# mathwrx/Decouple-and-Couple_Learning_in_Multi-Modal_Brain_Tumor_Segmentation

Measured on AMD Instinct MI355X. Metric: training volumes/sec (4x128^3), higher is better.
Workload: dtype bf16x3 forward (split-bf16 MFMA operands hi.hi+hi.lo+lo.hi: logits within 1e-3 of the fp32 reference) / bf16 data-gradient / bf16 weight-gradient MFMA operands; f32 accumulate, f32 storage, f32 master weights; 1 GPU; configs[1]: 1xMI355X, batch 2 per GPU, 4-modality 128^3 synthetic BraTS patches; fwd + softmax_dice + 4 sub-region/edge losses + bwd + Adam(amsgrad); random-init weights, dropout on; global_batch=2, parallelism=dp1, precision=bf16x3, dgrad_precision=bf16, wgrad_precision=bf16, mode=plan

## Files before the change

decouple-and-couple_learning_in_multi-modal_brain_tumor_segmentation_amd/csrc/gemm.hip:

```cpp
#include "common.h"
#include <cstdlib>

typedef struct cwf_gemm_args GemmArgs;


template <int TM, int TN, int GK>
__global__ __launch_bounds__(256) void gemm_mfma_kernel(const GemmArgs a) {
  constexpr int LDA_S = GK + 1, LDB_S = TN + 16;
  constexpr int IM = TM / 32, JN = TN / 32;
  constexpr int SA = TM * GK / 256, SB = TN * GK / 256;
  __shared__ float As[TM * LDA_S];
  __shared__ float Bs[GK * LDB_S];
  const int tid = threadIdx.x, lane = tid & 63, wave = tid >> 6;
  const int wr = wave >> 1, wc = wave & 1;
  const int r = lane & 15, kq = lane >> 4;
  const int zb = blockIdx.z / a.ZH, zh = blockIdx.z % a.ZH;
  const int m0 = blockIdx.y * TM, n0 = blockIdx.x * TN;
  const int64_t a_zoff = zb * a.sa_zb + zh * a.sa_zh;
  const float* A = ((a.A2 && n0 >= a.split_n) ? a.A2 : a.A) + a_zoff;
  const bool tabB = a.B_tab[0] != nullptr;
  const float* B = tabB ? a.B_tab[blockIdx.z] : a.B + zb * a.sb_zb + zh * a.sb_zh;
  if (a.B2 && m0 >= a.split_m) B = a.B2 + zb * a.sb_zb + zh * a.sb_zh;
  const bool a_drop = a.a_drop_p > 0.f;
  float* rowsum = a.rowsum_tab[0] ? a.rowsum_tab[blockIdx.z] : a.rowsum;
  const bool do_rs = rowsum != nullptr && blockIdx.x == 0 && wc == 0;

  f32x4 acc[IM][JN], accr[IM];
#pragma unroll
  for (int i = 0; i < IM; ++i) {
    accr[i] = (f32x4){0.f, 0.f, 0.f, 0.f};
#pragma unroll
    for (int j = 0; j < JN; ++j) acc[i][j] = (f32x4){0.f, 0.f, 0.f, 0.f};
  }

  const bool a_kfast = (a.sa_k == 1);
  const bool b_nfast = (a.sb_n == 1);
  int am[SA], ak[SA], bk[SB], bn[SB];
#pragma unroll
  for (int i = 0; i < SA; ++i) {
    if (a_kfast) { ak[i] = tid % GK; am[i] = tid / GK + (256 / GK) * i; } else { am[i] = tid % TM; ak[i] = tid / TM + (256 / TM) * i; }
  }
#pragma unroll
  for (int i = 0; i < SB; ++i) {
    if (b_nfast) { bn[i] = tid % TN; bk[i] = tid / TN + (256 / TN) * i; } else { bk[i] = tid % GK; bn[i] = tid / GK + (256 / GK) * i; }
  }
  float ra[SA], rb[SB];
  auto fetch = [&](int k0) {
#pragma unroll
    for (int i = 0; i < SA; ++i) {
      const int gm = m0 + am[i], gk = k0 + ak[i];
      float v = 0.f;
      if (gm < a.M && gk < a.K) {
        const int64_t off = gm * a.sa_m + gk * a.sa_k;
        v = A[off];
        if (a_drop) v *= cwf_keep(a.rng, a.a_drop_off, (uint64_t)(a_zoff + off), a.a_drop_n, a.a_drop_p, a.a_drop_p2);
      }
      ra[i] = v;
    }
#pragma unroll
    for (int i = 0; i < SB; ++i) {
      const int gn = n0 + bn[i], gkb = k0 + bk[i];
      rb[i] = (gn < a.N && gkb < a.K) ? B[gkb * a.sb_k + gn * a.sb_n] : 0.f;
    }
  };
  fetch(0);
  for (int k0 = 0; k0 < a.K; k0 += GK) {
    if (k0) __syncthreads();
#pragma unroll
    for (int i = 0; i < SA; ++i) As[am[i] * LDA_S + ak[i]] = ra[i];
#pragma unroll
    for (int i = 0; i < SB; ++i) Bs[bk[i] * LDB_S + bn[i]] = rb[i];
    __syncthreads();
    if (k0 + GK < a.K) fetch(k0 + GK);
#pragma unroll
    for (int kk = 0; kk < GK / 4; ++kk) {
      float av[IM], bv[JN];
#pragma unroll
      for (int i = 0; i < IM; ++i) av[i] = As[(wr * (TM / 2) + i * 16 + r) * LDA_S + kk * 4 + kq];
#pragma unroll
      for (int j = 0; j < JN; ++j) bv[j] = Bs[(kk * 4 + kq) * LDB_S + wc * (TN / 2) + j * 16 + r];
#pragma unroll
      for (int i = 0; i < IM; ++i)
#pragma unroll
        for (int j = 0; j < JN; ++j) acc[i][j] = __builtin_amdgcn_mfma_f32_16x16x4f32(av[i], bv[j], acc[i][j], 0, 0, 0);
      if (do_rs) {
#pragma unroll
        for (int i = 0; i < IM; ++i) accr[i] = __builtin_amdgcn_mfma_f32_16x16x4f32(av[i], 1.0f, accr[i], 0, 0, 0);
      }
    }
  }
  const int64_t c_zoff = zb * a.sc_zb + zh * a.sc_zh;
  float* C = a.C_tab[0] ? a.C_tab[blockIdx.z] : a.C + c_zoff;
  float* C2 = a.C2 ? a.C2 + c_zoff : nullptr;
  const float* bias = a.bias_tab[0] ? a.bias_tab[blockIdx.z] : a.bias;
  const float* R = a.residual ? a.residual + zb * a.sr_zb + zh * a.sr_zh : nullptr;
  const bool c_drop = a.c_drop_p > 0.f;
#pragma unroll
  for (int i = 0; i < IM; ++i)
#pragma unroll
    for (int j = 0; j < JN; ++j) {
      const int gn = n0 + wc * (TN / 2) + j * 16 + r;
      if (gn >= a.N) continue;
      const float bv = bias ? bias[gn] : 0.f;
#pragma unroll
      for (int e = 0; e < 4; ++e) {
        const int gm = m0 + wr * (TM / 2) + i * 16 + kq * 4 + e;
        if (gm >= a.M) continue;
        const int64_t off = gm * a.sc_m + gn;
        float v = acc[i][j][e] * a.alpha + bv;
        if (C2) C2[off] = v;
        if (a.act == 1) v = 0.5f * v * (1.f + erff(v * 0.70710678118654752440f));
        if (c_drop) v *= cwf_keep(a.rng, a.c_drop_off, (uint64_t)(c_zoff + off), a.c_drop_n, a.c_drop_p, a.c_drop_p2);
        if (R) v += R[gm * a.sr_m + gn];
        float* p = C + off;
        if (a.accumulate) v += *p;
        *p = v;
      }
    }
  if (do_rs && r == 0) {
#pragma unroll
    for (int i = 0; i < IM; ++i)
#pragma unroll
      for (int e = 0; e < 4; ++e) {
        const int gm = m0 + wr * (TM / 2) + i * 16 + kq * 4 + e;
        if (gm < a.M) rowsum[gm] = (a.rowsum_acc ? rowsum[gm] : 0.f) + accr[i][e];
      }
  }
}

template <int TM, int TN, int GK, bool AK, bool BN>
__global__ __launch_bounds__(256) void gemm_mfma_v_kernel(const GemmArgs a) {
  constexpr int LDA_S = GK + 1, LDB_S = TN + 16;
  constexpr int IM = TM / 32, JN = TN / 32;
  constexpr int SA = TM * GK / 1024, SB = TN * GK / 1024;
  __shared__ float As[TM * LDA_S];
  __shared__ __attribute__((aligned(16))) float Bs[GK * LDB_S];
  const int tid = threadIdx.x, lane = tid & 63, wave = tid >> 6;
  const int wr = wave >> 1, wc = wave & 1;
  const int r = lane & 15, kq = lane >> 4;
  const int zb = blockIdx.z / a.ZH, zh = blockIdx.z % a.ZH;
  const int m0 = blockIdx.y * TM, n0 = blockIdx.x * TN;
  const int64_t a_zoff = zb * a.sa_zb + zh * a.sa_zh;
  const float* A = ((a.A2 && n0 >= a.split_n) ? a.A2 : a.A) + a_zoff;
  const bool tabB = a.B_tab[0] != nullptr;
  const float* B = tabB ? a.B_tab[blockIdx.z] : a.B + zb * a.sb_zb + zh * a.sb_zh;
  if (a.B2 && m0 >= a.split_m) B = a.B2 + zb * a.sb_zb + zh * a.sb_zh;
  const bool a_drop = a.a_drop_p > 0.f;
  float* rowsum = a.rowsum_tab[0] ? a.rowsum_tab[blockIdx.z] : a.rowsum;
  const bool do_rs = rowsum != nullptr && blockIdx.x == 0 && wc == 0;

  f32x4 acc[IM][JN], accr[IM];
#pragma unroll
  for (int i = 0; i < IM; ++i) {
    accr[i] = (f32x4){0.f, 0.f, 0.f, 0.f};
#pragma unroll
    for (int j = 0; j < JN; ++j) acc[i][j] = (f32x4){0.f, 0.f, 0.f, 0.f};
  }
  int am[SA], ak[SA], bk[SB], bn[SB];
#pragma unroll
  for (int i = 0; i < SA; ++i) {
    if (AK) { ak[i] = (tid % (GK / 4)) * 4; am[i] = tid / (GK / 4) + (1024 / GK) * i; }
    else { am[i] = (tid % (TM / 4)) * 4; ak[i] = tid / (TM / 4) + (1024 / TM) * i; }
  }
#pragma unroll
  for (int i = 0; i < SB; ++i) {
    if (BN) { bn[i] = (tid % (TN / 4)) * 4; bk[i] = tid / (TN / 4) + (1024 / TN) * i; }
    else { bk[i] = (tid % (GK / 4)) * 4; bn[i] = tid / (GK / 4) + (1024 / GK) * i; }
  }
  f32x4 ra[SA], rb[SB];
  auto fetch = [&](int k0) {
#pragma unroll
    for (int i = 0; i < SA; ++i) {
      const int gm = m0 + am[i], gk = k0 + ak[i];
      f32x4 v = {0.f, 0.f, 0.f, 0.f};
      if (gm < a.M && gk < a.K) {
        const int64_t off = gm * a.sa_m + gk * a.sa_k;
        v = *reinterpret_cast<const f32x4*>(A + off);
        if (a_drop) {
          const int64_t st = AK ? 1 : a.sa_m;
#pragma unroll
          for (int c = 0; c < 4; ++c) v[c] *= cwf_keep(a.rng, a.a_drop_off, (uint64_t)(a_zoff + off + c * st), a.a_drop_n, a.a_drop_p, a.a_drop_p2);
        }
      }
      ra[i] = v;
    }
#pragma unroll
    for (int i = 0; i < SB; ++i) {
      const int gn = n0 + bn[i], gkb = k0 + bk[i];
      rb[i] = (gn < a.N && gkb < a.K) ? *reinterpret_cast<const f32x4*>(B + gkb * a.sb_k + gn * a.sb_n) : (f32x4){0.f, 0.f, 0.f, 0.f};
    }
  };
  fetch(0);
  for (int k0 = 0; k0 < a.K; k0 += GK) {
    if (k0) __syncthreads();
#pragma unroll
    for (int i = 0; i < SA; ++i)
#pragma unroll
      for (int c = 0; c < 4; ++c) {
        if (AK) As[am[i] * LDA_S + ak[i] + c] = ra[i][c];
        else As[(am[i] + c) * LDA_S + ak[i]] = ra[i][c];
      }
#pragma unroll
    for (int i = 0; i < SB; ++i) {
      if (BN) *reinterpret_cast<f32x4*>(&Bs[bk[i] * LDB_S + bn[i]]) = rb[i];
      else {
#pragma unroll
        for (int c = 0; c < 4; ++c) Bs[(bk[i] + c) * LDB_S + bn[i]] = rb[i][c];
      }
    }
    __syncthreads();
    if (k0 + GK < a.K) fetch(k0 + GK);
#pragma unroll
    for (int kk = 0; kk < GK / 4; ++kk) {
      float av[IM], bv[JN];
#pragma unroll
      for (int i = 0; i < IM; ++i) av[i] = As[(wr * (TM / 2) + i * 16 + r) * LDA_S + kk * 4 + kq];
#pragma unroll
      for (int j = 0; j < JN; ++j) bv[j] = Bs[(kk * 4 + kq) * LDB_S + wc * (TN / 2) + j * 16 + r];
#pragma unroll
      for (int i = 0; i < IM; ++i)
#pragma unroll
        for (int j = 0; j < JN; ++j) acc[i][j] = __builtin_amdgcn_mfma_f32_16x16x4f32(av[i], bv[j], acc[i][j], 0, 0, 0);
      if (do_rs) {
#pragma unroll
        for (int i = 0; i < IM; ++i) accr[i] = __builtin_amdgcn_mfma_f32_16x16x4f32(av[i], 1.0f, accr[i], 0, 0, 0);
      }
    }
  }
  const int64_t c_zoff = zb * a.sc_zb + zh * a.sc_zh;
  float* C = a.C_tab[0] ? a.C_tab[blockIdx.z] : a.C + c_zoff;
  float* C2 = a.C2 ? a.C2 + c_zoff : nullptr;
  const float* bias = a.bias_tab[0] ? a.bias_tab[blockIdx.z] : a.bias;
  const float* R = a.residual ? a.residual + zb * a.sr_zb + zh * a.sr_zh : nullptr;
  const bool c_drop = a.c_drop_p > 0.f;
#pragma unroll
  for (int i = 0; i < IM; ++i)
#pragma unroll
    for (int j = 0; j < JN; ++j) {
      const int gn = n0 + wc * (TN / 2) + j * 16 + r;
      if (gn >= a.N) continue;
      const float bv = bias ? bias[gn] : 0.f;
#pragma unroll
      for (int e = 0; e < 4; ++e) {
        const int gm = m0 + wr * (TM / 2) + i * 16 + kq * 4 + e;
        if (gm >= a.M) continue;
        const int64_t off = gm * a.sc_m + gn;
        float v = acc[i][j][e] * a.alpha + bv;
        if (C2) C2[off] = v;
        if (a.act == 1) v = 0.5f * v * (1.f + erff(v * 0.70710678118654752440f));
        if (c_drop) v *= cwf_keep(a.rng, a.c_drop_off, (uint64_t)(c_zoff + off), a.c_drop_n, a.c_drop_p, a.c_drop_p2);
        if (R) v += R[gm * a.sr_m + gn];
        float* p = C + off;
        if (a.accumulate) v += *p;
        *p = v;
      }
    }
  if (do_rs && r == 0) {
#pragma unroll
    for (int i = 0; i < IM; ++i)
#pragma unroll
      for (int e = 0; e < 4; ++e) {
        const int gm = m0 + wr * (TM / 2) + i * 16 + kq * 4 + e;
        if (gm < a.M) rowsum[gm] = (a.rowsum_acc ? rowsum[gm] : 0.f) + accr[i][e];
      }
  }
}

static bool gemm_vec_ok(const GemmArgs& a, bool* ak, bool* bn) {
  auto al = [](const void* p) { return (reinterpret_cast<uintptr_t>(p) & 15) == 0; };
  auto m4 = [](int64_t v) { return (v & 3) == 0; };
  if (!m4(a.sa_zb) || !m4(a.sa_zh) || !m4(a.sb_zb) || !m4(a.sb_zh)) return false;
  if (!al(a.A) || (a.A2 && !al(a.A2)) || (a.B && !al(a.B)) || (a.B2 && !al(a.B2))) return false;
  for (int z = 0; z < 4; ++z)
    if (a.B_tab[z] && !al(a.B_tab[z])) return false;
  if (a.sa_k == 1 && m4(a.K) && m4(a.sa_m)) *ak = true;
  else if (a.sa_m == 1 && m4(a.M) && m4(a.sa_k)) *ak = false;
  else return false;
  if (a.sb_n == 1 && m4(a.N) && m4(a.sb_k)) *bn = true;
  else if (a.sb_k == 1 && m4(a.K) && m4(a.sb_n)) *bn = false;
  else return false;
  if (a.B2 && (a.split_m & 3)) return false;
  return true;
}

struct GemmVariant { bool vec; int tm; bool ak, bn; };
static GemmVariant gemm_variant(const GemmArgs& a) {
  const int64_t wg64 = (int64_t)cdiv(a.N, 64) * cdiv(a.M, 64) * a.ZB * a.ZH;
  GemmVariant v = {false, wg64 >= 256 ? 64 : 32, false, false};
  if (a.K >= 64 && gemm_vec_ok(a, &v.ak, &v.bn)) v.vec = true;
  else v.ak = v.bn = false;
  return v;
}

static int gemm_check(const GemmArgs& a) {
  if (!a.A || (!a.B && !a.B_tab[0]) || (!a.C && !a.C_tab[0]) || a.M <= 0 || a.N <= 0 || a.K <= 0 || a.ZB <= 0 || a.ZH <= 0) return CWF_E_BADARG;
  if ((a.B_tab[0] || a.bias_tab[0] || a.C_tab[0] || a.rowsum_tab[0]) && (a.ZH != 1 || a.ZB > 4)) return CWF_E_BADARG;
  if ((int64_t)a.ZB * a.ZH > 65535) return CWF_E_TOOLARGE;
  if ((a.A2 && (a.split_n & 63)) || (a.B2 && (a.split_m & 63))) return CWF_E_BADARG;
  if ((a.a_drop_p > 0.f || a.c_drop_p > 0.f) && !a.rng) return CWF_E_BADARG;
  if (a.rowsum && (int64_t)a.ZB * a.ZH != 1) return CWF_E_BADARG;
  for (int z = 0; z < a.ZB && z < 4; ++z)
    if ((a.B_tab[0] && !a.B_tab[z]) || (a.bias_tab[0] && !a.bias_tab[z]) || (a.C_tab[0] && !a.C_tab[z]) || (a.rowsum_tab[0] && !a.rowsum_tab[z])) return CWF_E_BADARG;
  return 0;
}

extern "C" int cwf_gemm_ex(const struct cwf_gemm_args* args, void* stream) {
  if (!args) return CWF_E_BADARG;
  const GemmArgs& a = *args;
  const int rc = gemm_check(a);
  if (rc) return rc;
  const GemmVariant v = gemm_variant(a);
  const bool big = v.tm == 64;
  if (v.vec) {
    dim3 grid(cdiv(a.N, big ? 64 : 32), cdiv(a.M, big ? 64 : 32), a.ZB * a.ZH);
#define CWF_GV(AKv, BNv) do { if (big) hipLaunchKernelGGL((gemm_mfma_v_kernel<64, 64, 32, AKv, BNv>), grid, dim3(256), 0, cwf_stream(stream), a); \
                              else hipLaunchKernelGGL((gemm_mfma_v_kernel<32, 32, 64, AKv, BNv>), grid, dim3(256), 0, cwf_stream(stream), a); } while (0)
    if (v.ak && v.bn) CWF_GV(true, true); else if (v.ak) CWF_GV(true, false); else if (v.bn) CWF_GV(false, true); else CWF_GV(false, false);
#undef CWF_GV
    CWF_LAUNCH_CHECK();
    return 0;
  }
  if (big) {
    dim3 grid(cdiv(a.N, 64), cdiv(a.M, 64), a.ZB * a.ZH);
    hipLaunchKernelGGL((gemm_mfma_kernel<64, 64, 32>), grid, dim3(256), 0, cwf_stream(stream), a);
  } else {
    dim3 grid(cdiv(a.N, 32), cdiv(a.M, 32), a.ZB * a.ZH);
    hipLaunchKernelGGL((gemm_mfma_kernel<32, 32, 32>), grid, dim3(256), 0, cwf_stream(stream), a);
  }
  CWF_LAUNCH_CHECK();
  return 0;
}

extern "C" int cwf_debug_gemm_variant(const struct cwf_gemm_args* args, int* out) {
  if (!args || !out) return CWF_E_BADARG;
  const int rc = gemm_check(*args);
  if (rc) return rc;
  const GemmVariant v = gemm_variant(*args);
  out[0] = v.vec; out[1] = v.tm; out[2] = v.ak; out[3] = v.bn;
  return 0;
}

extern "C" int cwf_gemm(const float* A, int64_t sa_m, int64_t sa_k, int64_t sa_zb, int64_t sa_zh,
                        const float* B, int64_t sb_k, int64_t sb_n, int64_t sb_zb, int64_t sb_zh,
                        float* C, int64_t sc_m, int64_t sc_zb, int64_t sc_zh,
                        const float* bias, const float* residual, int64_t sr_m, int64_t sr_zb, int64_t sr_zh,
                        int M, int Nn, int K, int ZB, int ZH, float alpha, int act, int accumulate, void* stream) {
  GemmArgs a = {};
  a.A = A; a.sa_m = sa_m; a.sa_k = sa_k; a.sa_zb = sa_zb; a.sa_zh = sa_zh;
  a.B = B; a.sb_k = sb_k; a.sb_n = sb_n; a.sb_zb = sb_zb; a.sb_zh = sb_zh;
  a.C = C; a.sc_m = sc_m; a.sc_zb = sc_zb; a.sc_zh = sc_zh;
  a.bias = bias; a.residual = residual; a.sr_m = sr_m; a.sr_zb = sr_zb; a.sr_zh = sr_zh;
  a.M = M; a.N = Nn; a.K = K; a.ZB = ZB; a.ZH = ZH; a.alpha = alpha; a.act = act; a.accumulate = accumulate;
  return cwf_gemm_ex(&a, stream);
}

template <int PER>
__global__ __launch_bounds__(256) void layernorm_fwd_kernel(const float* __restrict__ x, const float* __restrict__ gamma, const float* __restrict__ beta,
                                                           float* __restrict__ y, float* __restrict__ mean, float* __restrict__ rstd, int rows, int E, float eps) {
  const int row = blockIdx.x * 4 + (threadIdx.x >> 6), lane = threadIdx.x & 63;
  if (row >= rows) return;
  const float* xr = x + (int64_t)row * E;
  float v[PER]; float s = 0.f;
#pragma unroll
  for (int i = 0; i < PER; ++i) { v[i] = xr[lane + 64 * i]; s += v[i]; }
  const float mu = wave_sum(s) / (float)E;
  float q = 0.f;
#pragma unroll
  for (int i = 0; i < PER; ++i) { const float d = v[i] - mu; q += d * d; }
  const float rs = rsqrtf(wave_sum(q) / (float)E + eps);
#pragma unroll
  for (int i = 0; i < PER; ++i) { const int c = lane + 64 * i; y[(int64_t)row * E + c] = (v[i] - mu) * rs * gamma[c] + beta[c]; }
  if (lane == 0) { mean[row] = mu; rstd[row] = rs; }
}

template <int PER>
__global__ __launch_bounds__(256) void layernorm_bwd_kernel(const float* __restrict__ dy, const float* __restrict__ x, const float* __restrict__ gamma,
                                                           const float* __restrict__ mean, const float* __restrict__ rstd, float* __restrict__ dx,
                                                           float* __restrict__ dgamma, float* __restrict__ dbeta, int rows, int E, int accumulate) {
  __shared__ float sg[4 * 64 * PER], sb[4 * 64 * PER];
  const int w = threadIdx.x >> 6, lane = threadIdx.x & 63;
  const int row = blockIdx.x * 4 + w;
  float pg[PER], pb[PER];
#pragma unroll
  for (int i = 0; i < PER; ++i) { pg[i] = 0.f; pb[i] = 0.f; }
  if (row < rows) {
    const float mu = mean[row], rs = rstd[row];
    float g[PER], h[PER]; float s1 = 0.f, s2 = 0.f;
#pragma unroll
    for (int i = 0; i < PER; ++i) {
      const int c = lane + 64 * i;
      const float d = dy[(int64_t)row * E + c];
// ... 351 lines not shown
```

decouple-and-couple_learning_in_multi-modal_brain_tumor_segmentation_amd/cwf/_lib.py:

```python
from __future__ import annotations

import ctypes as C
import os

_HERE = os.path.dirname(os.path.abspath(__file__))
LIB_PATH = os.path.join(_HERE, "libcwf_hip.so")

P = C.c_void_p
I = C.c_int
L = C.c_int64
F = C.c_float
U = C.c_uint32
U64 = C.c_uint64
D = C.c_double

SIGNATURES = {
    "cwf_version": [],
    "cwf_conv": [P, P],
    "cwf_conv_x16_ok": [I, I, I, I, I, I, I],
    "cwf_wgrad": [P, P, P],
    "cwf_gather_split_bf16": [P, I, L, P],
    "cwf_wgrad_nsplit": [I, I, I, I, I, I, I],
    "cwf_wgrad_partial_floats": [I, I, I, I, I, I, I],
    "cwf_wgrad_slab_floats": [I, I, I],
    "cwf_wgrad_reduce": [P, I, L, P, P, P, P],
    "cwf_gather_batched": [P, I, L, P],
    "cwf_in_finalize": [P, P, P, I, L, F, P],
    "cwf_in_stats": [P, I, P, I, L, I, P],
    "cwf_norm_act_add": [P, I, P, P, F, P, I, P, I, I, L, I, P],
    "cwf_in_bwd_stats": [P, I, P, I, P, P, F, P, I, L, I, P],
    "cwf_in_bwd_apply": [P, I, P, I, P, P, F, P, P, I, P, I, I, L, I, P],
    "cwf_in_bwd_apply_ex": [P, I, P, I, P, P, F, P, P, I, P, I, P, P, I, L, I, P],
    "cwf_norm_act_add_ex": [P, I, P, P, F, P, I, P, I, P, I, L, I, P],
    "cwf_to_bf16": [P, I, P, P, F, P, I, L, I, P],
    "cwf_gemm": [P, L, L, L, L, P, L, L, L, L, P, L, L, L, P, P, L, L, L, I, I, I, I, I, F, I, I, P],
    "cwf_layernorm_fwd": [P, P, P, P, P, P, I, I, F, P],
    "cwf_layernorm_bwd": [P, P, P, P, P, P, P, P, I, I, I, P],
    "cwf_softmax_rows": [P, L, I, I, P],
    "cwf_softmax_rows_bwd": [P, P, L, I, I, P],
    "cwf_gelu_bwd": [P, P, P, L, P],
    "cwf_colsum": [P, L, I, I, P, I, P],
    "cwf_window_to_tokens": [P, I, P, I, I, I, I, I, I, I, I, P],
    "cwf_tokens_to_window": [P, P, I, I, I, I, I, I, I, I, I, I, P],
    "cwf_token_scores": [P, P, L, P, I, I, I, P],
    "cwf_topk": [P, P, I, I, I, P],
    "cwf_gather_tokens": [P, P, P, L, P, F, P, I, I, I, I, P],
    "cwf_gather_tokens_bwd": [P, P, P, P, P, L, I, I, I, I, P],
    "cwf_scatter_rows": [P, P, P, L, L, P, L, P, I, I, I, I, P],
    "cwf_scatter_rows_bwd": [P, P, P, P, L, P, I, P, L, L, P, L, I, I, I, I, P],
    "cwf_upsample_softmax": [P, I, P, I, I, I, I, I, I, P],
    "cwf_upsample_softmax_bwd": [P, P, P, I, I, I, I, I, I, I, P, P],
    "cwf_channel_softmax": [P, I, P, L, I, P],
    "cwf_channel_softmax_bwd": [P, P, P, I, L, I, P],
    "cwf_dice_ce_sums": [P, P, U, P, I, L, I, P],
    "cwf_dice_ce_finalize": [P, P, P, I, L, I, P],
    "cwf_dice_ce_bwd": [P, P, U, P, P, P, I, L, I, P],
    "cwf_adam_amsgrad": [P, I, L, C.c_double, C.c_double, C.c_double, C.c_double, C.c_double, I, I, P, P],
    "cwf_adam_amsgrad_scaled": [P, I, L, C.c_double, C.c_double, C.c_double, C.c_double, C.c_double, I, I, P, F, P],
    "cwf_grad_add": [P, P, P, L, P],
    "cwf_grad_norm_clip": [P, L, F, F, P, P, P],
    "cwf_adam_amsgrad_ex": [P, I, L, C.c_double, C.c_double, C.c_double, C.c_double, C.c_double, I, I, P, F, P, P, F, P],
    "cwf_wgrad_reduce_batched": [P, I, P],
    "cwf_dropout_mask": [P, L, F, F, C.c_uint64, C.c_uint64, P],
    "cwf_mul": [P, P, P, L, P],
    "cwf_add": [P, P, P, L, P],
    "cwf_channel_scale": [P, I, P, P, I, I, L, I, P],
    "cwf_copy_strided": [P, I, P, I, L, I, P],
    "cwf_add3": [P, P, P, P, L, P],
    "cwf_bcast3": [P, P, L, P],
    "cwf_stats_channel_sum": [P, P, I, I, P],
    "cwf_gemm_ex": [P, P],
    "cwf_attn_fwd": [P, L, P, L, I, I, I, I, F, P, U64, F, P],
    "cwf_attn_bwd": [P, L, P, L, P, I, I, I, I, F, P, U64, F, P],
    "cwf_ln_pair_fwd": [P, P, I, P, P, P, P, P, P, P, I, I, F, P],
    "cwf_ln_pair_bwd": [P, P, P, P, P, I, P, P, P, P, P, P, P, P, P, I, I, I, P],
    "cwf_gelu_bwd_drop": [P, P, P, L, P, U64, F, P],
    "cwf_token_scores2": [P, P, L, P, L, P, P, I, I, I, P],
    "cwf_topk_inv": [P, P, P, P, P, P, I, I, I, P],
    "cwf_index_inv": [P, P, I, I, I, P],
    "cwf_gather_multi": [P, I, I, I, I, F, P, F, P],
    "cwf_scatter_inv": [P, P, P, L, L, P, L, P, P, I, I, I, P],
    "cwf_scatter_bwd": [P, P, P, P, P, P, L, L, P, L, P, L, P, L, L, P, L, I, I, I, I, P],
    "cwf_token_grad": [P, P, P, L, P, P, P, L, P, L, P, U64, U64, F, P, I, I, I, I, P],
    "cwf_head_grad": [P, P, P, P, L, P, P, I, I, P],
    "cwf_dice_ce_finalize_multi": [P, P, P, P, I, I, L, I, P],
    "cwf_head_loss_sums": [P, I, I, P, P, P, I, I, I, I, I, P],
    "cwf_head_loss_bwd": [P, I, I, P, P, P, P, P, I, P, I, I, I, I, I, P],
    "cwf_head_loss_bwd_ex": [P, I, I, P, P, P, P, P, I, I, P, I, I, I, I, I, P],
    "cwf_ln_pair_fwd_g": [P, P, I, P, I, P, P, P, I, I, F, P],
    "cwf_ln_pair_bwd_g": [P, P, P, P, P, I, P, I, P, P, P, I, I, I, P],
    "cwf_token_scores2_g": [P, P, P, I, I, P, P, I, I, I, P],
    "cwf_head_grad_g": [P, P, P, P, L, P, P, I, I, I, P],
    "cwf_window_to_tokens_g": [P, I, P, I, I, I, I, I, I, I, I, I, P],
    "cwf_tokens_to_window_g": [P, P, I, I, I, I, I, I, I, I, I, I, P],
    "cwf_cat3_channels": [P, P, P, P, L, I, P],
    "cwf_stitch_windows": [P, P, I, P],
    "cwf_argmax_dice": [P, L, L, L, P, P, P, I, L, P],
    "cwf_argmax_metrics": [P, L, L, L, P, P, P, I, L, P],
    "cwf_region_bits": [P, P, L, P],
    "cwf_hausdorff_workspace": [I, I, I, I, I],
    "cwf_hausdorff": [P, P, I, I, I, I, I, D, D, D, I, I, P, P, P, P, L, P],
    "cwf_surface_metrics_workspace": [I, I, I, I, I],
    "cwf_surface_metrics": [P, P, I, I, I, I, I, D, D, D, I, I, P, I, P, P, P, P, P, P, P, P, L, P],
    "cwf_components_workspace": [I, I, I, I, I],
    "cwf_components": [P, I, I, I, I, I, I, P, P, P, P, P, L, P],
    "cwf_postprocess_labels": [P, P, P, P, P, I, I, I, I, I, I, I, I, I, I, I, I, P, P, P],
    "cwf_label_metrics": [P, P, P, L, P],
    "cwf_dilate_bits": [P, P, I, I, I, I, I, I, P, L, P],
    "cwf_lesionwise_workspace": [I, I, I, I, I],
    "cwf_lesionwise": [P, P, I, I, I, I, I, I, L, D, P, P, P, P, P, P, L, P],
    "cwf_lesionwise_ex_workspace": [I, I, I, I, I],
    "cwf_lesionwise_ex": [P, P, I, I, I, I, I, I, L, D, P, I, P, P, P, P, P, P, P, P, L, P],
    "cwf_prepare_batch": [P, I, I, I, I, P, L, P, L, P, L, P],
    "cwf_prepare_batch_affine": [P, I, I, I, I, P, L, P, L, P, L, P],
    "cwf_prepare_batch_elastic": [P, I, I, I, I, P, L, P, L, P, L, P],
    "cwf_augment_intensity": [P, I, I, I, I, P, L, P, L, P, L, P],
    "cwf_augment_acquisition": [P, I, I, I, I, P, L, P, L, P, L, P],
    "cwf_window_gather": [P, P, P, I, I, P],
    "cwf_window_blend": [P, P, P, P, I, I, I, P],
    "cwf_window_finalize": [P, P, P, P, P],
    "cwf_normalize_nonzero": [P, L, P, P],
    "cwf_rng_advance": [P, P],
    "cwf_dropout_mask_rng": [P, L, F, F, P, U64, P],
    "cwf_plan_create": [P, P],
# ... 138 lines not shown
```

include/cwf_hip.h:

```cpp
#ifndef CWF_HIP_H
#define CWF_HIP_H
#include <stdint.h>
#ifdef __cplusplus
extern "C" {
#endif

#define CWF_E_BADARG   (-1)
#define CWF_E_TOOLARGE (-2)
#define CWF_E_ALIGN    (-3)

int cwf_version(void);
const char* cwf_arch(void);

enum { CWF_CONV3_S1 = 0, CWF_CONV3_S2 = 1, CWF_CONV1 = 2, CWF_CONVT2 = 3, CWF_CONV3_S2_DGRAD = 4, CWF_CONVT2_DGRAD = 5 };
enum { CWF_FP32 = 0, CWF_BF16X3 = 1, CWF_BF16 = 2 };

struct cwf_conv_args {
  int op, precision;
  const float* x; int x_ldc; const void* wpk; const float* bias; float* y; int y_ldc;
  const float* in_scale; const float* in_shift; float in_slope;
  const float* residual; int r_ldc; const float* out_scale; double* stats;
  const float* nb_x; int nb_ldc; const float* nb_scale; const float* nb_shift; float nb_slope;
  const void* x16; const void* zero16; void* y16;
  const float* w_raw;
// ... 15 lines not shown
  int groups; const float* x_g[3]; const float* dy_g[3]; float* partial_g[3];
  int N, Di, Hi, Wi, Cin, Do, Ho, Wo, Cout;
};
int cwf_wgrad(const struct cwf_wgrad_args* args , int* nsplit_used , void* stream);
int cwf_wgrad_reduce(const float* partial, int nsplit, int64_t slab_floats,
                     const int32_t* inv_map, float* dW, float* db, void* stream);
struct cwf_wgrad_reduce_desc { const float* partial; const int32_t* inv; float* dW; float* db; int64_t slab; int32_t nsplit; int32_t pad_; };
int cwf_wgrad_reduce_batched(const struct cwf_wgrad_reduce_desc* table, int nlayers, void* stream);

struct cwf_gather_desc { const float* src; float* dst; const int32_t* map; int64_t n; };

int cwf_gather_split_bf16(const struct cwf_gather_desc* table, int nlayers, int64_t max_n, void* stream);

int cwf_gather_batched(const struct cwf_gather_desc* table, int nlayers, int64_t max_n, void* stream);

int cwf_in_finalize(const double* stats, float* scale, float* shift, int NC, int64_t V, float eps, void* stream);
int cwf_in_stats(const float* x, int x_ldc, double* stats, int N, int64_t V, int C, void* stream);
int cwf_norm_act_add(const float* x, int x_ldc, const float* scale, const float* shift, float slope,
                     const float* residual, int r_ldc, float* y, int y_ldc, int N, int64_t V, int C, void* stream);
int cwf_in_bwd_stats(const float* dy, int dy_ldc, const float* x, int x_ldc, const float* scale, const float* shift,
                     float slope, double* sums, int N, int64_t V, int C, void* stream);
int cwf_in_bwd_apply(const float* dy, int dy_ldc, const float* x, int x_ldc, const float* scale, const float* shift,
                     float slope, const double* sums, const float* dx_add, int a_ldc, float* dx, int dx_ldc,
                     int N, int64_t V, int C, void* stream);

int cwf_in_bwd_apply_ex(const float* dy, int dy_ldc, const float* x, int x_ldc, const float* scale, const float* shift,
                        float slope, const double* sums, const float* dx_add, int a_ldc, float* dx, int dx_ldc,
                        void* dx16, void* xa16, int N, int64_t V, int C, void* stream);
int cwf_norm_act_add_ex(const float* x, int x_ldc, const float* scale, const float* shift, float slope,
                        const float* residual, int r_ldc, float* y, int y_ldc, void* y16, int N, int64_t V, int C, void* stream);
int cwf_to_bf16(const float* x, int x_ldc, const float* scale, const float* shift, float slope, void* y16,
                int N, int64_t V, int C, void* stream);
int cwf_gemm(const float* A, int64_t sa_m, int64_t sa_k, int64_t sa_zb, int64_t sa_zh,
             const float* B, int64_t sb_k, int64_t sb_n, int64_t sb_zb, int64_t sb_zh,
             float* C, int64_t sc_m, int64_t sc_zb, int64_t sc_zh,
             const float* bias, const float* residual, int64_t sr_m, int64_t sr_zb, int64_t sr_zh,
             int M, int Nn, int K, int ZB, int ZH, float alpha, int act, int accumulate, void* stream);
struct cwf_gemm_args {
  const float* A; int64_t sa_m, sa_k, sa_zb, sa_zh;
  const float* B; int64_t sb_k, sb_n, sb_zb, sb_zh;
  float* C; int64_t sc_m, sc_zb, sc_zh;
  const float* bias; const float* residual; int64_t sr_m, sr_zb, sr_zh;
  int M, N, K, ZB, ZH; float alpha; int act; int accumulate;
  const float* A2; int split_n;
  const float* B2; int split_m;
  float* C2;
  float* rowsum; int rowsum_acc;
  const uint64_t* rng;
  uint64_t a_drop_off, a_drop_n; float a_drop_p, a_drop_p2;
  uint64_t c_drop_off, c_drop_n; float c_drop_p, c_drop_p2;
  const float* B_tab[4]; const float* bias_tab[4]; float* C_tab[4]; float* rowsum_tab[4];
};
int cwf_gemm_ex(const struct cwf_gemm_args* args , void* stream);

int cwf_attn_fwd(const float* qkv, int64_t ld, float* o, int64_t ldo, int Z, int T, int E, int heads, float scale,
                 const uint64_t* rng, uint64_t drop_off, float drop_p, void* stream);
int cwf_attn_bwd(const float* qkv, int64_t ld, const float* d_o, int64_t ldo, float* dqkv, int Z, int T, int E, int heads,
                 float scale, const uint64_t* rng, uint64_t drop_off, float drop_p, void* stream);

int cwf_ln_pair_fwd(const float* x, const float* x2, int perm_T, const float* g1, const float* b1, const float* g2, const float* b2,
                    float* ya, float* yb, float* stats, int rows, int E, float eps, void* stream);
struct cwf_ln_group_params { const float* g1[4]; const float* b1[4]; const float* g2[4]; const float* b2[4];
                             float* dg1[4]; float* db1[4]; float* dg2[4]; float* db2[4]; };
int cwf_ln_pair_fwd_g(const float* x, const float* x2, int perm_T, const struct cwf_ln_group_params* h_params, int groups,
                      float* ya, float* yb, float* stats, int rows, int E, float eps, void* stream);
int cwf_ln_pair_bwd_g(const float* dy, const float* da, const float* db, const float* x, const float* x2, int perm_T,
                      const struct cwf_ln_group_params* h_params, int groups, const float* stats, float* dx, float* dx2,
                      int rows, int E, int accumulate_params, void* stream);
int cwf_ln_pair_bwd(const float* dy, const float* da, const float* db, const float* x, const float* x2, int perm_T,
                    const float* g1, const float* g2, const float* stats, float* dx, float* dx2,
                    float* dg1, float* db1, float* dg2, float* db2, int rows, int E, int accumulate_params, void* stream);
int cwf_gelu_bwd_drop(const float* z, const float* dh, float* dz, int64_t n, const uint64_t* rng, uint64_t off, float p, void* stream);

int cwf_layernorm_fwd(const float* x, const float* gamma, const float* beta, float* y, float* mean, float* rstd,
                      int rows, int E, float eps, void* stream);
int cwf_layernorm_bwd(const float* dy, const float* x, const float* gamma, const float* mean, const float* rstd,
                      float* dx, float* dgamma, float* dbeta, int rows, int E, int accumulate, void* stream);
int cwf_softmax_rows(float* s, int64_t rows, int cols, int ld, void* stream);
int cwf_softmax_rows_bwd(const float* p, float* dp_inout, int64_t rows, int cols, int ld, void* stream);
int cwf_gelu_bwd(const float* x, const float* dy, float* dx, int64_t n, void* stream);
int cwf_colsum(const float* x, int64_t rows, int cols, int ld, float* out, int accumulate, void* stream);

int cwf_window_to_tokens(const float* x, int x_ldc, float* tok, int B, int D, int H, int W, int C,
                         int p0, int p1, int p2, void* stream);
int cwf_tokens_to_window(const float* tok, float* x, int x_ldc, int B, int D, int H, int W, int C,
                         int p0, int p1, int p2, int accumulate, void* stream);
int cwf_token_scores(const float* feats, const float* query, int64_t query_bstride, float* score,
                     int B, int T, int E, void* stream);
int cwf_topk(const float* score, int32_t* index, int B, int T, int k, void* stream);
int cwf_gather_tokens(const float* feats, const int32_t* index, const float* head, int64_t head_bstride,
                      const float* keep, float pe_odd, float* seq, int B, int T, int k, int E, void* stream);
int cwf_gather_tokens_bwd(const float* dseq, const int32_t* index, const float* keep, float* dfeats, float* dhead,
                          int64_t dhead_bstride, int B, int T, int k, int E, void* stream);
int cwf_scatter_rows(const float* feats, const int32_t* index, const float* rows, int64_t rows_ld, int64_t rows_bs,
                     const float* gate, int64_t gate_bs, float* out, int B, int T, int k, int E, void* stream);
int cwf_scatter_rows_bwd(const float* dout, const int32_t* index, const float* scat, const float* gate, int64_t gate_bs,
                         float* dfeats, int accumulate, float* drows, int64_t drows_ld, int64_t drows_bs,
                         float* dgate, int64_t dgate_bs, int B, int T, int k, int E, void* stream);

int cwf_token_scores2(const float* feats, const float* q1, int64_t q1_bstride, const float* q2, int64_t q2_bstride,
                      float* s1, float* s2, int B, int T, int E, void* stream);
int cwf_token_scores2_g(const float* feats, const float* const* h_q1, const float* const* h_q2, int groups, int group_B,
                        float* s1, float* s2, int B, int T, int E, void* stream);
int cwf_topk_inv(const float* score0, int32_t* index0, int32_t* inv0, const float* score1, int32_t* index1, int32_t* inv1,
                 int B, int T, int k, void* stream);
int cwf_index_inv(const int32_t* index, int32_t* inv, int B, int T, int k, void* stream);
// ... 188 lines not shown
```

Baseline: 117.2 volumes/s.

## Add warp-specialized DMA GEMM with triple-buffered global-to-LDS loads

Adds a GEMM kernel in which dedicated loader waves stream A/B tiles straight into LDS through global_load_lds into a 3-stage ring with swizzled layout. Compute waves run fp32 MFMA with software-pipelined LDS reads, and a tile-index remap groups blocks across XCDs. It is routed only for vectorizable GEMMs whose tile count is mid-sized, to overlap memory latency with compute. The epilogue and operand setup are factored into shared helpers. The cost is extra barriers, larger LDS use and more waves per block, plus the risk of vmcnt/barrier ordering bugs.

After: 118.1 volumes/s, median of 6. Within noise of the previous version (+0.8%).

```diff
diff --git a/decouple-and-couple_learning_in_multi-modal_brain_tumor_segmentation_amd/csrc/gemm.hip b/decouple-and-couple_learning_in_multi-modal_brain_tumor_segmentation_amd/csrc/gemm.hip
--- a/decouple-and-couple_learning_in_multi-modal_brain_tumor_segmentation_amd/csrc/gemm.hip
+++ b/decouple-and-couple_learning_in_multi-modal_brain_tumor_segmentation_amd/csrc/gemm.hip
@@ -1,8 +1,64 @@
 #include "common.h"
 #include <cstdlib>
+#include <type_traits>
 
 typedef struct cwf_gemm_args GemmArgs;
 
+
+struct GemmOperands { const float* A; const float* B; int64_t a_zoff; float* rowsum; };
+__device__ __forceinline__ GemmOperands gemm_operands(const GemmArgs& a, int m0, int n0, int zb, int zh, int z) {
+  GemmOperands o;
+  o.a_zoff = zb * a.sa_zb + zh * a.sa_zh;
+  o.A = ((a.A2 && n0 >= a.split_n) ? a.A2 : a.A) + o.a_zoff;
+  const bool tabB = a.B_tab[0] != nullptr;
+  o.B = tabB ? a.B_tab[z] : a.B + zb * a.sb_zb + zh * a.sb_zh;
+  if (a.B2 && m0 >= a.split_m) o.B = a.B2 + zb * a.sb_zb + zh * a.sb_zh;
+  o.rowsum = a.rowsum_tab[0] ? a.rowsum_tab[z] : a.rowsum;
+  return o;
+}
+
+template <int TM, int TN>
+__device__ __forceinline__ void gemm_epilogue(const GemmArgs& a, const f32x4 (&acc)[TM / 32][TN / 32], const f32x4 (&accr)[TM / 32],
+                                              int m0, int n0, int zb, int zh, int z, int wr, int wc, int r, int kq, float* rowsum, bool do_rs) {
+  constexpr int IM = TM / 32, JN = TN / 32;
+  const int64_t c_zoff = zb * a.sc_zb + zh * a.sc_zh;
+  float* C = a.C_tab[0] ? a.C_tab[z] : a.C + c_zoff;
+  float* C2 = a.C2 ? a.C2 + c_zoff : nullptr;
+  const float* bias = a.bias_tab[0] ? a.bias_tab[z] : a.bias;
+  const float* R = a.residual ? a.residual + zb * a.sr_zb + zh * a.sr_zh : nullptr;
+  const bool c_drop = a.c_drop_p > 0.f;
+#pragma unroll
+  for (int i = 0; i < IM; ++i)
+#pragma unroll
+    for (int j = 0; j < JN; ++j) {
+      const int gn = n0 + wc * (TN / 2) + j * 16 + r;
+      if (gn >= a.N) continue;
+      const float bv = bias ? bias[gn] : 0.f;
+#pragma unroll
+      for (int e = 0; e < 4; ++e) {
+        const int gm = m0 + wr * (TM / 2) + i * 16 + kq * 4 + e;
+        if (gm >= a.M) continue;
+        const int64_t off = gm * a.sc_m + gn;
+        float v = acc[i][j][e] * a.alpha + bv;
+        if (C2) C2[off] = v;
+        if (a.act == 1) v = 0.5f * v * (1.f + erff(v * 0.70710678118654752440f));
+        if (c_drop) v *= cwf_keep(a.rng, a.c_drop_off, (uint64_t)(c_zoff + off), a.c_drop_n, a.c_drop_p, a.c_drop_p2);
+        if (R) v += R[gm * a.sr_m + gn];
+        float* p = C + off;
+        if (a.accumulate) v += *p;
+        *p = v;
+      }
+    }
+  if (do_rs && r == 0) {
+#pragma unroll
+    for (int i = 0; i < IM; ++i)
+#pragma unroll
+      for (int e = 0; e < 4; ++e) {
+        const int gm = m0 + wr * (TM / 2) + i * 16 + kq * 4 + e;
+        if (gm < a.M) rowsum[gm] = (a.rowsum_acc ? rowsum[gm] : 0.f) + accr[i][e];
+      }
+  }
+}
 
 template <int TM, int TN, int GK>
 __global__ __launch_bounds__(256) void gemm_mfma_kernel(const GemmArgs a) {
@@ -16,13 +72,10 @@
   const int r = lane & 15, kq = lane >> 4;
   const int zb = blockIdx.z / a.ZH, zh = blockIdx.z % a.ZH;
   const int m0 = blockIdx.y * TM, n0 = blockIdx.x * TN;
-  const int64_t a_zoff = zb * a.sa_zb + zh * a.sa_zh;
-  const float* A = ((a.A2 && n0 >= a.split_n) ? a.A2 : a.A) + a_zoff;
-  const bool tabB = a.B_tab[0] != nullptr;
-  const float* B = tabB ? a.B_tab[blockIdx.z] : a.B + zb * a.sb_zb + zh * a.sb_zh;
-  if (a.B2 && m0 >= a.split_m) B = a.B2 + zb * a.sb_zb + zh * a.sb_zh;
+  const GemmOperands op = gemm_operands(a, m0, n0, zb, zh, blockIdx.z);
+  const float* A = op.A; const float* B = op.B; const int64_t a_zoff = op.a_zoff;
   const bool a_drop = a.a_drop_p > 0.f;
-  float* rowsum = a.rowsum_tab[0] ? a.rowsum_tab[blockIdx.z] : a.rowsum;
+  float* rowsum = op.rowsum;
   const bool do_rs = rowsum != nullptr && blockIdx.x == 0 && wc == 0;
 
   f32x4 acc[IM][JN], accr[IM];
@@ -89,43 +142,7 @@
       }
     }
   }
-  const int64_t c_zoff = zb * a.sc_zb + zh * a.sc_zh;
-  float* C = a.C_tab[0] ? a.C_tab[blockIdx.z] : a.C + c_zoff;
-  float* C2 = a.C2 ? a.C2 + c_zoff : nullptr;
-  const float* bias = a.bias_tab[0] ? a.bias_tab[blockIdx.z] : a.bias;
-  const float* R = a.residual ? a.residual + zb * a.sr_zb + zh * a.sr_zh : nullptr;
-  const bool c_drop = a.c_drop_p > 0.f;
-#pragma unroll
-  for (int i = 0; i < IM; ++i)
-#pragma unroll
-    for (int j = 0; j < JN; ++j) {
-      const int gn = n0 + wc * (TN / 2) + j * 16 + r;
-      if (gn >= a.N) continue;
-      const float bv = bias ? bias[gn] : 0.f;
-#pragma unroll
-      for (int e = 0; e < 4; ++e) {
-        const int gm = m0 + wr * (TM / 2) + i * 16 + kq * 4 + e;
-        if (gm >= a.M) continue;
-        const int64_t off = gm * a.sc_m + gn;
-        float v = acc[i][j][e] * a.alpha + bv;
-        if (C2) C2[off] = v;
-        if (a.act == 1) v = 0.5f * v * (1.f + erff(v * 0.70710678118654752440f));
-        if (c_drop) v *= cwf_keep(a.rng, a.c_drop_off, (uint64_t)(c_zoff + off), a.c_drop_n, a.c_drop_p, a.c_drop_p2);
-        if (R) v += R[gm * a.sr_m + gn];
-        float* p = C + off;
-        if (a.accumulate) v += *p;
-        *p = v;
-      }
-    }
-  if (do_rs && r == 0) {
-#pragma unroll
-    for (int i = 0; i < IM; ++i)
-#pragma unroll
-      for (int e = 0; e < 4; ++e) {
-        const int gm = m0 + wr * (TM / 2) + i * 16 + kq * 4 + e;
-        if (gm < a.M) rowsum[gm] = (a.rowsum_acc ? rowsum[gm] : 0.f) + accr[i][e];
-      }
-  }
+  gemm_epilogue<TM, TN>(a, acc, accr, m0, n0, zb, zh, blockIdx.z, wr, wc, r, kq, rowsum, do_rs);
 }
 
 template <int TM, int TN, int GK, bool AK, bool BN>
@@ -140,13 +157,10 @@
   const int r = lane & 15, kq = lane >> 4;
   const int zb = blockIdx.z / a.ZH, zh = blockIdx.z % a.ZH;
   const int m0 = blockIdx.y * TM, n0 = blockIdx.x * TN;
-  const int64_t a_zoff = zb * a.sa_zb + zh * a.sa_zh;
-  const float* A = ((a.A2 && n0 >= a.split_n) ? a.A2 : a.A) + a_zoff;
-  const bool tabB = a.B_tab[0] != nullptr;
-  const float* B = tabB ? a.B_tab[blockIdx.z] : a.B + zb * a.sb_zb + zh * a.sb_zh;
-  if (a.B2 && m0 >= a.split_m) B = a.B2 + zb * a.sb_zb + zh * a.sb_zh;
+  const GemmOperands op = gemm_operands(a, m0, n0, zb, zh, blockIdx.z);
+  const float* A = op.A; const float* B = op.B; const int64_t a_zoff = op.a_zoff;
   const bool a_drop = a.a_drop_p > 0.f;
-  float* rowsum = a.rowsum_tab[0] ? a.rowsum_tab[blockIdx.z] : a.rowsum;
+  float* rowsum = op.rowsum;
   const bool do_rs = rowsum != nullptr && blockIdx.x == 0 && wc == 0;
 
   f32x4 acc[IM][JN], accr[IM];
@@ -227,43 +241,169 @@
       }
     }
   }
-  const int64_t c_zoff = zb * a.sc_zb + zh * a.sc_zh;
-  float* C = a.C_tab[0] ? a.C_tab[blockIdx.z] : a.C + c_zoff;
-  float* C2 = a.C2 ? a.C2 + c_zoff : nullptr;
-  const float* bias = a.bias_tab[0] ? a.bias_tab[blockIdx.z] : a.bias;
-  const float* R = a.residual ? a.residual + zb * a.sr_zb + zh * a.sr_zh : nullptr;
-  const bool c_drop = a.c_drop_p > 0.f;
-#pragma unroll
-  for (int i = 0; i < IM; ++i)
-#pragma unroll
-    for (int j = 0; j < JN; ++j) {
-      const int gn = n0 + wc * (TN / 2) + j * 16 + r;
-      if (gn >= a.N) continue;
-      const float bv = bias ? bias[gn] : 0.f;
-#pragma unroll
-      for (int e = 0; e < 4; ++e) {
-        const int gm = m0 + wr * (TM / 2) + i * 16 + kq * 4 + e;
-        if (gm >= a.M) continue;
-        const int64_t off = gm * a.sc_m + gn;
-        float v = acc[i][j][e] * a.alpha + bv;
-        if (C2) C2[off] = v;
-        if (a.act == 1) v = 0.5f * v * (1.f + erff(v * 0.70710678118654752440f));
-        if (c_drop) v *= cwf_keep(a.rng, a.c_drop_off, (uint64_t)(c_zoff + off), a.c_drop_n, a.c_drop_p, a.c_drop_p2);
-        if (R) v += R[gm * a.sr_m + gn];
-        float* p = C + off;
-        if (a.accumulate) v += *p;
-        *p = v;
-      }
-    }
-  if (do_rs && r == 0) {
-#pragma unroll
-    for (int i = 0; i < IM; ++i)
-#pragma unroll
-      for (int e = 0; e < 4; ++e) {
-        const int gm = m0 + wr * (TM / 2) + i * 16 + kq * 4 + e;
-        if (gm < a.M) rowsum[gm] = (a.rowsum_acc ? rowsum[gm] : 0.f) + accr[i][e];
-      }
-  }
+  gemm_epilogue<TM, TN>(a, acc, accr, m0, n0, zb, zh, blockIdx.z, wr, wc, r, kq, rowsum, do_rs);
+}
+
+#define GD_T 64
+#define GD_K 64
+#define GD_S 3
+#define GD_LW 4
+#define GD_OPB (GD_T * GD_K * 4)
+#define GD_BUFB (2 * GD_OPB)
+#define GD_LDS (GD_S * GD_BUFB)
+typedef __attribute__((address_space(3))) void* gd_lds_vp;
+typedef __attribute__((address_space(1))) const void* gd_glb_vp;
+__device__ float4 gd_zero16 = {0.f, 0.f, 0.f, 0.f};
+
+template <bool KF> __device__ __forceinline__ int gd_src_granule(int row, int pc) { return KF ? (pc ^ (row & 15)) : (pc ^ ((row & 3) << 2)); }
+
+template <bool AK, bool BN, bool ADROP>
+__device__ __forceinline__ void gemm_dma_loader(const GemmArgs& a, const float* A, const float* B, int m0, int n0, unsigned lds_base,
+                                                int lw, int lane, int nsteps) {
+  constexpr int NI = 2 * (GD_T * GD_K / 256) / GD_LW;
+  static_assert(NI == 8 && GD_S == 3, "the vmcnt immediates below leave one step of NI pieces in flight");
+  int64_t off[NI]; int kl[NI]; bool okx[NI];
+#pragma unroll
+  for (int i = 0; i < NI; ++i) {
+    const bool isB = i >= NI / 2;
+    const int p = lw * (NI / 2) + (i & (NI / 2 - 1));
+    const int row = 4 * p + (lane >> 4), pc = lane & 15;
+    if (!isB) {
+      const int c = gd_src_granule<AK>(row, pc);
+      if (AK) { const int gm = m0 + row; off[i] = gm * a.sa_m + 4 * c; kl[i] = 4 * c; okx[i] = gm < a.M; }
+      else { const int gm = m0 + 4 * c; off[i] = row * a.sa_k + gm; kl[i] = row; okx[i] = gm < a.M; }
+    } else {
+      const int c = gd_src_granule<!BN>(row, pc);
+      if (!BN) { const int gn = n0 + row; off[i] = gn * a.sb_n + 4 * c; kl[i] = 4 * c; okx[i] = gn < a.N; }
+      else { const int gn = n0 + 4 * c; off[i] = row * a.sb_k + gn; kl[i] = row; okx[i] = gn < a.N; }
+    }
+  }
+  const int64_t stepA = AK ? GD_K : GD_K * a.sa_k, stepB = BN ? GD_K * a.sb_k : GD_K;
+  const float* zero = reinterpret_cast<const float*>(&gd_zero16);
+  auto issue = [&](int it, int buf) __attribute__((always_inline)) {
+    const int k0 = it * GD_K;
+    const unsigned lbuf = lds_base + (unsigned)buf * GD_BUFB;
+#pragma unroll
+    for (int i = 0; i < NI; ++i) {
+      const bool isB = i >= NI / 2;
+      const int p = lw * (NI / 2) + (i & (NI / 2 - 1));
+      const bool ok = okx[i] && k0 + kl[i] < a.K;
+      const int64_t o = ok ? off[i] + it * (isB ? stepB : stepA) : 0;
+      const float* src = ok ? (isB ? B : A) + o : zero;
+      __builtin_amdgcn_global_load_lds((gd_glb_vp)src, (gd_lds_vp)(uintptr_t)(lbuf + (isB ? GD_OPB : 0) + (unsigned)p * 1024u), 16, 0, 0);
+    }
+  };
+  if (nsteps > 0) issue(0, 0);
+  if (nsteps > 1) issue(1, 1);
+  int buf = 2;
+  for (int it = 0; it < nsteps; ++it) {
+    if (it + 1 < nsteps) asm volatile("s_waitcnt vmcnt(%0)" :: "n"(NI) : "memory");
+    else asm volatile("s_waitcnt vmcnt(0)" ::: "memory");
+    asm volatile("s_barrier" ::: "memory");
+    if (it + 2 < nsteps) issue(it + 2, buf);
+    buf = buf == GD_S - 1 ? 0 : buf + 1;
+    if (ADROP) asm volatile("s_barrier" ::: "memory");
+  }
+}
+
+template <bool AK, bool BN, bool ADROP>
+__global__ __launch_bounds__(256 + 64 * GD_LW) void gemm_dma_kernel(const GemmArgs a) {
+  extern __shared__ float4 gd_lds4[];
+  const int tid = threadIdx.x, lane = tid & 63;
+  const int wave = __builtin_amdgcn_readfirstlane(tid >> 6);
+  int z, m0, n0;
+  {
+    const int b = blockIdx.x, G = gridDim.x, x = b & 7;
+    const int t = x * (G >> 3) + min(x, G & 7) + (b >> 3);
+    const int nx = (a.N + GD_T - 1) / GD_T, ny = (a.M + GD_T - 1) / GD_T;
+    n0 = (t % nx) * GD_T; m0 = ((t / nx) % ny) * GD_T; z = t / (nx * ny);
+  }
+  const int zb = z / a.ZH, zh = z % a.ZH;
+  const GemmOperands op = gemm_operands(a, m0, n0, zb, zh, z);
+  const int nsteps = (a.K + GD_K - 1) / GD_K;
+  const unsigned lds_base = (unsigned)(uintptr_t)(__attribute__((address_space(3))) void*)gd_lds4;
+  if (wave >= 4) {
+    gemm_dma_loader<AK, BN, ADROP>(a, op.A, op.B, m0, n0, lds_base, wave - 4, lane, nsteps);
+    return;
+  }
+  const int wr = wave >> 1, wc = wave & 1;
+  const int r = lane & 15, kq = lane >> 4;
+  float* rowsum = op.rowsum;
+  const bool do_rs = rowsum != nullptr && n0 == 0 && wc == 0;
+  f32x4 acc[2][2], accr[2];
+#pragma unroll
+  for (int i = 0; i < 2; ++i) {
+    accr[i] = (f32x4){0.f, 0.f, 0.f, 0.f};
+#pragma unroll
+    for (int j = 0; j < 2; ++j) acc[i][j] = (f32x4){0.f, 0.f, 0.f, 0.f};
+  }
+  const char* lds = reinterpret_cast<const char*>(gd_lds4);
+  int fa[2], fb[2];
+#pragma unroll
+  for (int i = 0; i < 2; ++i) {
+    const int row = wr * 32 + i * 16 + r;
+    fa[i] = AK ? row * 256 + (r << 4) + kq * 4 : kq * 256 + ((((row >> 2) ^ (kq << 2))) << 4) + (r & 3) * 4;
+    const int col = wc * 32 + i * 16 + r;
+    fb[i] = !BN ? col * 256 + (r << 4) + kq * 4 : kq * 256 + ((((col >> 2) ^ (kq << 2))) << 4) + (r & 3) * 4;
+  }
+  int buf = 0;
+  for (int it = 0; it < nsteps; ++it) {
+    asm volatile("s_waitcnt lgkmcnt(0)\n\ts_barrier" ::: "memory");
+    const char* At = lds + buf * GD_BUFB;
+    const char* Bt = At + GD_OPB;
+    if (ADROP) {
+      float* Aw = reinterpret_cast<float*>(const_cast<char*>(At));
+      const int k0 = it * GD_K;
+#pragma unroll
+      for (int q = 0; q < 4; ++q) {
+        const int G = tid + 256 * q, row = G >> 4, c = gd_src_granule<AK>(row, G & 15);
+        const int gm = m0 + (AK ? row : 4 * c), gk = k0 + (AK ? 4 * c : row);
+        if (gm < a.M && gk < a.K) {
+          const int64_t off = gm * a.sa_m + gk * a.sa_k;
+          const int64_t st = AK ? 1 : a.sa_m;
+          f32x4 v = *reinterpret_cast<const f32x4*>(Aw + G * 4);
+#pragma unroll
+          for (int e = 0; e < 4; ++e) v[e] *= cwf_keep(a.rng, a.a_drop_off, (uint64_t)(op.a_zoff + off + e * st), a.a_drop_n, a.a_drop_p, a.a_drop_p2);
+          *reinterpret_cast<f32x4*>(Aw + G * 4) = v;
+        }
+      }
+      asm volatile("s_waitcnt lgkmcnt(0)\n\ts_barrier" ::: "memory");
+    }
+    auto kstep = [&](auto rs) __attribute__((always_inline)) {
+      float av[2][4][2], bv[2][4][2];
+      auto rd = [&](int set, int b) __attribute__((always_inline)) {
+#pragma unroll
+        for (int q = 0; q < 4; ++q) {
+          const int kk = 4 * b + q;
+#pragma unroll
+          for (int i = 0; i < 2; ++i) av[set][q][i] = *reinterpret_cast<const float*>(At + (AK ? (fa[i] ^ (kk << 4)) : fa[i] + kk * 1024));
+#pragma unroll
+          for (int j = 0; j < 2; ++j) bv[set][q][j] = *reinterpret_cast<const float*>(Bt + (!BN ? (fb[j] ^ (kk << 4)) : fb[j] + kk * 1024));
+        }
+      };
+      rd(0, 0);
+#pragma unroll
+      for (int b = 0; b < GD_K / 16; ++b) {
+        if (b + 1 < GD_K / 16) rd((b + 1) & 1, b + 1);
+        __builtin_amdgcn_sched_barrier(0);
+#pragma unroll
+        for (int q = 0; q < 4; ++q) {
+#pragma unroll
+          for (int i = 0; i < 2; ++i)
+#pragma unroll
+            for (int j = 0; j < 2; ++j) acc[i][j] = __builtin_amdgcn_mfma_f32_16x16x4f32(av[b & 1][q][i], bv[b & 1][q][j], acc[i][j], 0, 0, 0);
+          if (decltype(rs)::value) {
+#pragma unroll
+            for (int i = 0; i < 2; ++i) accr[i] = __builtin_amdgcn_mfma_f32_16x16x4f32(av[b & 1][q][i], 1.0f, accr[i], 0, 0, 0);
+          }
+        }
+        __builtin_amdgcn_sched_barrier(0);
+      }
+    };
+    if (do_rs) kstep(std::true_type{}); else kstep(std::false_type{});
+    buf = buf == GD_S - 1 ? 0 : buf + 1;
+  }
+  gemm_epilogue<GD_T, GD_T>(a, acc, accr, m0, n0, zb, zh, z, wr, wc, r, kq, rowsum, do_rs);
 }
 
 static bool gemm_vec_ok(const GemmArgs& a, bool* ak, bool* bn) {
@@ -292,6 +432,16 @@
   return v;
 }
 
+static int g_gemm_dma = 1;
+static bool gemm_dma_takes(const GemmArgs& a, const GemmVariant& v) {
+  if (g_gemm_dma == 0 || !v.vec) return false;
+  if (g_gemm_dma == 2) return true;
+  const int64_t tiles = (int64_t)cdiv(a.N, 64) * cdiv(a.M, 64) * a.ZB * a.ZH;
+  if (tiles < 96 || tiles > 256) return false;
+  if (a.a_drop_p > 0.f && !v.ak) return false;
+  return true;
+}
+
 static int gemm_check(const GemmArgs& a) {
   if (!a.A || (!a.B && !a.B_tab[0]) || (!a.C && !a.C_tab[0]) || a.M <= 0 || a.N <= 0 || a.K <= 0 || a.ZB <= 0 || a.ZH <= 0) return CWF_E_BADARG;
   if ((a.B_tab[0] || a.bias_tab[0] || a.C_tab[0] || a.rowsum_tab[0]) && (a.ZH != 1 || a.ZB > 4)) return CWF_E_BADARG;
@@ -311,6 +461,18 @@
   if (rc) return rc;
   const GemmVariant v = gemm_variant(a);
   const bool big = v.tm == 64;
+  if (gemm_dma_takes(a, v)) {
+    dim3 grid(cdiv(a.N, GD_T) * cdiv(a.M, GD_T) * a.ZB * a.ZH);
+    const bool ad = a.a_drop_p > 0.f;
+#define CWF_GD(AKv, BNv, ADv) do { CWF_MAX_LDS_ONCE((&gemm_dma_kernel<AKv, BNv, ADv>)); \
+                                   hipLaunchKernelGGL((gemm_dma_kernel<AKv, BNv, ADv>), grid, dim3(256 + 64 * GD_LW), GD_LDS, cwf_stream(stream), a); } while (0)
+#define CWF_GD2(AKv, BNv) do { if (ad) CWF_GD(AKv, BNv, true); else CWF_GD(AKv, BNv, false); } while (0)
+    if (v.ak && v.bn) CWF_GD2(true, true); else if (v.ak) CWF_GD2(true, false); else if (v.bn) CWF_GD2(false, true); else CWF_GD2(false, false);
+#undef CWF_GD2
+#undef CWF_GD
+    CWF_LAUNCH_CHECK();
+    return 0;
+  }
   if (v.vec) {
     dim3 grid(cdiv(a.N, big ? 64 : 32), cdiv(a.M, big ? 64 : 32), a.ZB * a.ZH);
 #define CWF_GV(AKv, BNv) do { if (big) hipLaunchKernelGGL((gemm_mfma_v_kernel<64, 64, 32, AKv, BNv>), grid, dim3(256), 0, cwf_stream(stream), a); \
@@ -337,6 +499,16 @@
   if (rc) return rc;
   const GemmVariant v = gemm_variant(*args);
   out[0] = v.vec; out[1] = v.tm; out[2] = v.ak; out[3] = v.bn;
+  return 0;
+}
+
+extern "C" int cwf_debug_gemm_dma(int on) { const int old = g_gemm_dma; g_gemm_dma = on; return old; }
+
+extern "C" int cwf_debug_gemm_route(const struct cwf_gemm_args* args, int* out) {
+  if (!args || !out) return CWF_E_BADARG;
+  const int rc = gemm_check(*args);
+  if (rc) return rc;
+  out[0] = gemm_dma_takes(*args, gemm_variant(*args)); out[1] = GD_T; out[2] = GD_S; out[3] = args->a_drop_p > 0.f;
   return 0;
 }
 
diff --git a/decouple-and-couple_learning_in_multi-modal_brain_tumor_segmentation_amd/cwf/_lib.py b/decouple-and-couple_learning_in_multi-modal_brain_tumor_segmentation_amd/cwf/_lib.py
--- a/decouple-and-couple_learning_in_multi-modal_brain_tumor_segmentation_amd/cwf/_lib.py
+++ b/decouple-and-couple_learning_in_multi-modal_brain_tumor_segmentation_amd/cwf/_lib.py
@@ -70,6 +70,8 @@
     "cwf_bcast3": [P, P, L, P],
     "cwf_stats_channel_sum": [P, P, I, I, P],
     "cwf_gemm_ex": [P, P],
+    "cwf_debug_gemm_dma": [I],
+    "cwf_debug_gemm_route": [P, P],
     "cwf_attn_fwd": [P, L, P, L, I, I, I, I, F, P, U64, F, P],
     "cwf_attn_bwd": [P, L, P, L, P, I, I, I, I, F, P, U64, F, P],
     "cwf_ln_pair_fwd": [P, P, I, P, P, P, P, P, P, P, I, I, F, P],
diff --git a/include/cwf_hip.h b/include/cwf_hip.h
--- a/include/cwf_hip.h
+++ b/include/cwf_hip.h
@@ -91,6 +91,8 @@
   const float* B_tab[4]; const float* bias_tab[4]; float* C_tab[4]; float* rowsum_tab[4];
 };
 int cwf_gemm_ex(const struct cwf_gemm_args* args , void* stream);
+int cwf_debug_gemm_dma(int on);
+int cwf_debug_gemm_route(const struct cwf_gemm_args* args , int* out);
 
 int cwf_attn_fwd(const float* qkv, int64_t ld, float* o, int64_t ldo, int Z, int T, int E, int heads, float scale,
                  const uint64_t* rng, uint64_t drop_off, float drop_p, void* stream);
```
